# skovaka/UNCALLED

Hardware: AMD Instinct MI355X
Metric: reads_mapped_per_sec (higher is better)
Workload: dtype u64+f32/f64; 1 GPU; E. coli 4.6 Mb synthetic ref (ecoli_syn seed 1), synthetic r9.4.1 reads (3600 bases ~ 32k samples, 10% off-target), all reference defaults; batches_in_flight=2, remapped_reads=0, parallelism=reads sharded over 1 GPU(s), index replicated

## Files before the change

__graft_entry__.py:

```python
import os
import shutil
import subprocess
import sys
from pathlib import Path

ROOT = Path(__file__).resolve().parent
PKG = ROOT / "uncalled_amd"
CSRC = PKG / "csrc"
LIB = ROOT / "uncalled_amd" / "libuncalled_hip.so"
HIP_SOURCES = ["k_events.hip", "k_map.hip", "k_taps.hip", "k_sort.hip", "k_dtw.hip", "k_align.hip", "unc_host.cpp", "unc_dtw.cpp",
               "unc_align.cpp"]
HIPCC_FLAGS = ["--offload-arch=gfx950", "-O3", "-std=c++17", "-ffp-contract=off",
               "-fno-gpu-flush-denormals-to-zero", "-fPIC", "-shared", "-x", "hip"]


def _hipcc():
    for cand in (shutil.which("hipcc"), "/opt/rocm/bin/hipcc"):
        if cand and Path(cand).exists():
            return cand
    raise RuntimeError("hipcc not found")


def _stale(target, sources):
    if not target.exists():
        return True
    t = target.stat().st_mtime
# ... 93 lines not shown
```

include/uncalled_hip.h:

```cpp
#ifndef UNCALLED_HIP_H
#define UNCALLED_HIP_H
#include <stddef.h>
#include <stdint.h>

#ifdef __cplusplus
extern "C" {
#endif

typedef enum {
    UNC_OK = 0,
    UNC_ERR_ARG = -1,
    UNC_ERR_IO = -2,
    UNC_ERR_HIP = -3,
    UNC_ERR_NOMEM = -4,
    UNC_ERR_OVERFLOW = -5
} unc_status_t;

#define UNC_SEED_LEN 22
#define UNC_KLEN 5
#define UNC_NKMER 1024
#define UNC_WINDOW1 3
#define UNC_WINDOW2 6

typedef struct {
// ... 236 lines not shown
    unc_dtw_result_t dtw;
    uint32_t n_events, n_kept;
    float tgt_mean, tgt_stdv;
    float scale, shift;
    uint32_t status, pad;
} unc_align_result_t;
int unc_align_batch(int device, const unc_params_t *params, const unc_align_opts_t *opts, uint32_t n_reads, const int16_t *raw,
                    const uint64_t *offsets, const unc_calib_t *calib, int on_device, uint32_t n_queries, const unc_align_query_t *queries,
                    const uint16_t *kmers, const uint64_t *km_off, uint64_t workspace_bytes, unc_align_result_t *results, float *levels,
                    const uint64_t *lev_off, uint32_t *path, const uint64_t *path_off, void *stream);
int unc_align_last_timing(float *ms4);
void unc_align_model_target(float *mean, float *stdv);

int unc_calib_traffic(int device, uint64_t n_records, int reps);
int unc_calib_chase(int device, const void *base, uint64_t bytes, uint32_t waves, uint32_t steps, float *ms_out);

int unc_detect_events(unc_mapper_t *m, uint32_t n_reads, const int16_t *raw, const uint64_t *offsets,
                      const unc_calib_t *calib, float *means, uint64_t means_cap, uint64_t *means_offsets,
                      unc_evt_info_t *info);
int unc_trace_begin(unc_mapper_t *m, const int16_t *raw, uint32_t n, const unc_calib_t *calib);
int unc_trace_step(unc_mapper_t *m, uint32_t n_events , int *done);
int unc_trace_paths(unc_mapper_t *m, unc_path_t *out, uint32_t cap, uint32_t *n_out);
int unc_trace_clusters(unc_mapper_t *m, unc_cluster_t *out, uint32_t cap, uint32_t *n_out, unc_cluster_t *max_map,
                       float *len_sum, uint32_t *n_lens);
int unc_trace_finish(unc_mapper_t *m, unc_hit_t *hit);

#ifdef __cplusplus
}
#endif
#endif
// ... 1 lines not shown
```

uncalled_amd/csrc/unc_host.cpp:

```cpp
#include <hip/hip_runtime.h>

#include <math.h>
#include <stdarg.h>
#include <stdio.h>
#include <stdlib.h>
#include <string.h>

#include <string>
#include <chrono>
#include <algorithm>
#include <array>
#include <map>
#include <mutex>
#include <utility>
#include <vector>

#include "r94_model_table.h"
#include "unc_dev_types.h"
#include "unc_kernels.h"
#include "unc_host_util.h"

using namespace unc;

static thread_local char g_err[1024] = "";
// ... 128 lines not shown
        if (!fgets(line, sizeof line, fp)) line[0] = 0;
        long long off; int len, n_ambs;
        if (fscanf(fp, "%lld%d%d", &off, &len, &n_ambs) != 3) { fclose(fp); return fail(UNC_ERR_IO, "bad record in %s", fn.c_str()); }
        ix->seqs.push_back(SeqAnn{name, (uint64_t)off, (uint64_t)len});
    }
    fclose(fp);
    return UNC_OK;
}

extern "C" void unc_index_free(unc_index_t *ix) {
    if (!ix) return;
    (void)hipSetDevice(ix->device);
    delete ix;
}

struct PlacementSpacer {
    void *p = nullptr;
    size_t bytes = 0;
    explicit PlacementSpacer(size_t need_after) {
        size_t cap = 64ull << 30;
        if (const char *e = getenv("UNC_PLACEMENT_SPACER_GB")) cap = (size_t)strtoull(e, nullptr, 10) << 30;
        if (need_after < (1ull << 30)) return;
        size_t free_b = 0, total_b = 0;
        if (!cap || hipMemGetInfo(&free_b, &total_b) != hipSuccess) { (void)hipGetLastError(); return; }
        const size_t margin = 16ull << 30;
        if (free_b <= need_after + margin) return;
        const size_t want = std::min(cap, free_b - need_after - margin);
        if (want < (2ull << 30)) return;
        if (hipMalloc(&p, want) != hipSuccess) { p = nullptr; (void)hipGetLastError(); return; }
        bytes = want;
    }
    void release() { if (p) { (void)hipFree(p); p = nullptr; bytes = 0; } }
    ~PlacementSpacer() { release(); }
    PlacementSpacer(const PlacementSpacer &) = delete;
    PlacementSpacer &operator=(const PlacementSpacer &) = delete;
};

extern "C" int unc_index_load(const char *bwa_prefix, const char *idx_preset, int device, unc_index_t **out) {
    if (!bwa_prefix || !out) return fail(UNC_ERR_ARG, "null argument");
    *out = nullptr;
    std::string prefix(bwa_prefix);
    unc_index *ix = new unc_index();
    ix->device = device;
    struct Guard { unc_index *p; ~Guard() { if (p) unc_index_free(p); } } guard{ix};

    std::vector<char> bwt;
    if (!read_file(prefix + ".bwt", bwt) || bwt.size() < 40) return fail(UNC_ERR_IO, "failed to load BWA index: %s.bwt", bwa_prefix);
    memcpy(&ix->primary, bwt.data(), 8);
    memcpy(&ix->L2[1], bwt.data() + 8, 32);
    ix->seq_len = ix->L2[4];
    const size_t n_words = (bwt.size() - 40) / 4;
    const uint64_t n = ix->seq_len;
// ... 6 lines not shown
    memcpy(&sa_primary, sa.data(), 8);
    memcpy(&sa_intv, sa.data() + 40, 8);
    memcpy(&sa_seq_len, sa.data() + 48, 8);
    if (sa_primary != ix->primary || sa_seq_len != n || sa_intv != 32) return fail(UNC_ERR_IO, "%s.sa does not match the .bwt (interval must be 32)", bwa_prefix);
    const uint64_t n_sa = (n + 32) / 32;
    if (sa.size() != 56 + (n_sa - 1) * 8) return fail(UNC_ERR_IO, "%s.sa: unexpected size", bwa_prefix);

    int rc = parse_ann(prefix + ".ann", ix);
    if (rc) return rc;
    rc = parse_uncl(prefix + ".uncl", idx_preset ? idx_preset : "default", ix->thresholds);
    if (rc) return rc;
    build_model(ix);

    HIPCHK(hipSetDevice(device));
    const size_t bwt_bytes = ((n_words * 4 + 63) / 64 + 1) * 64;
    PlacementSpacer spacer(bwt_bytes + n_sa * 8 + ((size_t)n_words * 16 + 2) / 2 * 12 + (size_t)n_words * 2 + (64u << 20));
    HIPCHK(ix->d_bwt.alloc(bwt_bytes / 4));
    HIPCHK(hipMemset(ix->d_bwt.p, 0, bwt_bytes));
    HIPCHK(hipMemcpy(ix->d_bwt.p, bwt.data() + 40, n_words * 4, hipMemcpyHostToDevice));
    HIPCHK(ix->d_sa.alloc(n_sa));
    {
        std::vector<uint64_t> h(n_sa);
        h[0] = ~0ull;
        memcpy(h.data() + 1, sa.data() + 56, (n_sa - 1) * 8);
        HIPCHK(hipMemcpy(ix->d_sa.p, h.data(), n_sa * 8, hipMemcpyHostToDevice));
    }
    HIPCHK(ix->d_kmer_ranges.alloc(2 * NKMER));
    HIPCHK(ix->d_model.alloc(3 * NKMER));
    HIPCHK(hipMemcpy(ix->d_model.p, ix->model.data(), 3 * NKMER * 4, hipMemcpyHostToDevice));
    {
        std::vector<float> m4(4 * NKMER, 0.0f);
        for (int k = 0; k < NKMER; ++k) { m4[4 * k] = ix->model[k]; m4[4 * k + 1] = ix->model[NKMER + k]; m4[4 * k + 2] = ix->model[2 * NKMER + k]; }
        HIPCHK(ix->d_model4.alloc(4 * NKMER));
        HIPCHK(hipMemcpy(ix->d_model4.p, m4.data(), 4 * NKMER * 4, hipMemcpyHostToDevice));
    }
    ix->device_bytes = bwt_bytes + n_sa * 8 + 2 * NKMER * 8 + 3 * NKMER * 4;

    DevIndex &d = ix->dev;
    d.bwt = ix->d_bwt.p; d.sa = ix->d_sa.p; d.kmer_ranges = ix->d_kmer_ranges.p; d.model = ix->d_model.p; d.model4 = ix->d_model4.p;
    d.primary = ix->primary; d.seq_len = n;
    for (int i = 0; i < 5; ++i) d.L2[i] = ix->L2[i];
    memcpy(d.thresholds, ix->thresholds, sizeof d.thresholds);

    d.sa_dense = nullptr;
    {
        const char *env = getenv("UNC_DENSE_SA");
        size_t free_b = 0, total_b = 0;
        (void)hipMemGetInfo(&free_b, &total_b);
        free_b += spacer.bytes;
        const size_t need = ((n + 2) / 2) * 12 + 16;
        if (!(env && env[0] == '0') && need < free_b / 2) {
            HIPCHK(ix->d_sa_dense.alloc(need));
            uint64_t *const dense = reinterpret_cast<uint64_t *>(ix->d_sa_dense.p);
            launch_dense_sa(d, dense, nullptr);
            HIPCHK(hipGetLastError());
            HIPCHK(hipDeviceSynchronize());
            {
                DevBuf<uint32_t> d_bad;
                uint32_t bad = 0;
                HIPCHK(d_bad.alloc(1));
                HIPCHK(hipMemset(d_bad.p, 0, 4));
                launch_dense_sa_check(d, dense, 16384, d_bad.p, nullptr);
                HIPCHK(hipGetLastError());
                HIPCHK(hipMemcpy(&bad, d_bad.p, 4, hipMemcpyDeviceToHost));
                if (bad) return fail(UNC_ERR_HIP, "dense SA self-check failed on %u of 16384 probe rows", bad);
            }
            d.sa_dense = dense;
            ix->device_bytes += need;
        }
    }
    d.fm32 = nullptr;
    const char *fm32_env = getenv("UNC_FM32");
    if (n < 0xFFFFFF00ull && !(fm32_env && fm32_env[0] == '0')) {
        const uint32_t n_blk = (uint32_t)((n + 63) / 64 + 1);
        HIPCHK(ix->d_fm32.alloc((size_t)n_blk * 8));
        launch_build_fm32(d, ix->d_fm32.p, n_blk, nullptr);
        HIPCHK(hipGetLastError());
        HIPCHK(hipDeviceSynchronize());
        d.fm32 = ix->d_fm32.p;
        DevBuf<uint32_t> d_bad;
        uint32_t bad = 0;
        HIPCHK(d_bad.alloc(1));
        HIPCHK(hipMemset(d_bad.p, 0, 4));
        launch_fm32_check(d, 16384, d_bad.p, nullptr);
        HIPCHK(hipGetLastError());
        HIPCHK(hipMemcpy(&bad, d_bad.p, 4, hipMemcpyDeviceToHost));
        if (bad) return fail(UNC_ERR_HIP, "32-bit rank table self-check failed on %u of 16384 probe steps", bad);
        ix->device_bytes += (size_t)n_blk * 32;
    }
    launch_kmer_ranges(d, ix->d_kmer_ranges.p, nullptr);
// ... 118 lines not shown
    HIPCHK(l.alloc(n)); HIPCHK(o.alloc((size_t)n * NKMER));
    HIPCHK(hipMemcpy(l.p, levels, n * 4, hipMemcpyHostToDevice));
    launch_match_probs(ix->dev, n, l.p, o.p, nullptr);
    HIPCHK(hipGetLastError());
    HIPCHK(hipDeviceSynchronize());
    HIPCHK(hipMemcpy(out, o.p, (size_t)n * NKMER * 4, hipMemcpyDeviceToHost));
    return UNC_OK;
}

struct Scratch { DevBuf<char> mem; DevScratch v{}; };
struct Pool { DevBuf<char> nodes; DevBuf<PoolQueue> q; DevBuf<SchedCell> cells; DevPool v{}; };
struct Sched { DevBuf<SchedCtl> ctl; DevBuf<SchedCell> free_cells, park_cells; DevSched v{}; };

struct unc_mapper {
    const unc_index *ix = nullptr;
    unc_params_t P;
    uint32_t n_slots = 0, n_waves = 0, slice_events = 1024, ev_rpw = 64;
    Sched sched;
    Scratch sc;
    uint64_t device_bytes = 0;
    hipStream_t stream = nullptr;
    hipEvent_t ev[3] = {nullptr, nullptr, nullptr};
    double win_start_ms = 0, win_end_ms = 0;
    float ms_events = 0, ms_map = 0;
    double wave_busy = 0;
    float wall_khz = 0;
    bool profile = false;
    Pool pool;
    bool pool_auto = false;
    uint32_t pool_floor = 16, pool_created = 0, pool_hw_last = 0, pool_hw_max = 0, pool_resizes = 0;
// ... 58 lines not shown
    if (off >= (1ull << 32)) return fail(UNC_ERR_ARG, "per-read scratch of %llu bytes does not fit 32-bit offsets (max_clusters %u)", (unsigned long long)off, max_clusters);
    sc.off_paths = (uint32_t)o_paths; sc.off_levels = (uint32_t)o_levels; sc.off_order = (uint32_t)o_order; sc.off_keys = (uint32_t)o_keys;
    sc.off_seedp = (uint32_t)o_seedp; sc.off_tasks = (uint32_t)o_tasks; sc.off_cl_dir = (uint32_t)o_cld; sc.off_cl_chunks = (uint32_t)o_clc;
    sc.off_state = (uint32_t)o_state;
    sc.off_streams = (uint32_t)o_streams; sc.off_info = (uint32_t)o_info; sc.off_tmp = (uint32_t)o_tmp;
    sc.slot_bytes = off;
    return UNC_OK;
}

static uint64_t scratch_slot_bytes(const unc_params_t &P, uint32_t max_clusters, uint32_t max_seed_paths, const DevIndex &dix) {
    DevScratch t;
    return scratch_layout(t, P, max_clusters, max_seed_paths, dix) == UNC_OK ? t.slot_bytes : ~0ull;
}

static int alloc_scratch(Scratch &s, const unc_params_t &P, size_t n_slots, uint32_t max_clusters, uint32_t max_seed_paths,
                         size_t *bytes_out, const DevIndex &dix) {
    DevScratch &sc = s.v;
    int rc = scratch_layout(sc, P, max_clusters, max_seed_paths, dix);
    if (rc) return rc;
    const size_t bytes = (size_t)n_slots * sc.slot_bytes;
    HIPCHK(s.mem.alloc(bytes));
    sc.base = s.mem.p;
    HIPCHK(hipMemset2D(sc.base + sc.off_state, sc.slot_bytes, 0, sizeof(SlotState), n_slots));
    if (bytes_out) *bytes_out = bytes;
    return UNC_OK;
}

static uint32_t xcd_count(int device) {
    static std::mutex mu;
    static std::map<int, uint32_t> known;
    std::lock_guard<std::mutex> lk(mu);
    auto it = known.find(device);
    if (it != known.end()) return it->second;
    uint32_t n = 1;
    DevBuf<uint32_t> d;
    constexpr uint32_t NB = 256;
// ... 5 lines not shown
            for (uint32_t i = 0; i < NB; ++i) seen |= 1u << (h[i] & 15u);
            n = (uint32_t)__builtin_popcount(seen);
            if (seen != (n >= 32 ? ~0u : (1u << n) - 1u)) n = 1;
        }
    }
    (void)hipGetLastError();
    known[device] = n;
    return n;
}

static int alloc_pool(Pool &p, uint32_t n_chunks, size_t *bytes_out) {
    p = Pool{};
    uint32_t cap = 64;
    while (cap < n_chunks) cap <<= 1;
    p.v.cap_mask = cap - 1; p.v.n_chunks = n_chunks;
    HIPCHK(p.nodes.alloc((size_t)n_chunks * POOL_CHUNK_BYTES));
    HIPCHK(p.q.alloc(1));
    HIPCHK(p.cells.alloc(cap));
    p.v.nodes = p.nodes.p; p.v.q = p.q.p; p.v.cells = p.cells.p;
    launch_pool_init(p.v, nullptr);
    HIPCHK(hipGetLastError());
    HIPCHK(hipDeviceSynchronize());
    if (bytes_out) *bytes_out += (size_t)n_chunks * POOL_CHUNK_BYTES + (size_t)cap * sizeof(SchedCell);
    return UNC_OK;
}

static SlotState *slot_state(const DevScratch &sc, size_t slot) { return reinterpret_cast<SlotState *>(sc.base + slot * sc.slot_bytes + sc.off_state); }

extern "C" void unc_mapper_free(unc_mapper_t *m) {
    if (!m) return;
    (void)hipSetDevice(m->ix->device);
    for (auto &e : m->ev) if (e) (void)hipEventDestroy(e);
    if (m->stream) (void)hipStreamDestroy(m->stream);
    delete m;
}

static hipEvent_t g_ref_event = nullptr;
static std::mutex g_ref_mutex;
static int ref_event(hipEvent_t *out) {
    std::lock_guard<std::mutex> lock(g_ref_mutex);
    if (!g_ref_event) {
        HIPCHK(hipEventCreate(&g_ref_event));
        HIPCHK(hipEventRecord(g_ref_event, nullptr));
        HIPCHK(hipEventSynchronize(g_ref_event));
    }
    *out = g_ref_event;
    return UNC_OK;
}
extern "C" int unc_mapper_create(const unc_index_t *ix, const unc_params_t *p, const unc_mapper_opts_t *opts, unc_mapper_t **out) {
    if (!ix || !p || !out) return fail(UNC_ERR_ARG, "null argument");
    *out = nullptr;
    if (p->seed_len != UNC_SEED_LEN) return fail(UNC_ERR_ARG, "seed_len must be %d", UNC_SEED_LEN);
    if (p->window_length1 != UNC_WINDOW1 || p->window_length2 != UNC_WINDOW2) return fail(UNC_ERR_ARG, "event windows must be %d/%d", UNC_WINDOW1, UNC_WINDOW2);
    if (p->max_paths == 0 || p->max_paths > 65535) return fail(UNC_ERR_ARG, "max_paths must be in 1..65535");
    if (p->max_rep_copy > (uint32_t)MAX_REP_COPY_LIMIT) return fail(UNC_ERR_ARG, "max_rep_copy must be <= %d", MAX_REP_COPY_LIMIT);
    if (p->max_consec_stay > 255) return fail(UNC_ERR_ARG, "max_consec_stay must be <= 255");
    if (p->max_events > 65535) return fail(UNC_ERR_ARG, "max_events must be <= 65535");
    HIPCHK(hipSetDevice(ix->device));
    unc_mapper *m = new unc_mapper();
    struct Guard { unc_mapper *p; ~Guard() { if (p) unc_mapper_free(p); } } guard{m};
    m->ix = ix;
    m->P = *p;
    uint32_t n_slots = opts ? opts->n_slots : 0, n_waves = opts ? opts->n_waves : 0;
    if (n_waves == 0) {
        hipDeviceProp_t prop;
        HIPCHK(hipGetDeviceProperties(&prop, ix->device));
        n_waves = (uint32_t)prop.multiProcessorCount * map_kernel_waves_per_cu();
        if (n_slots && n_slots < n_waves) n_waves = n_slots;
    }
    if (n_slots == 0) {
        size_t free_b = 0, total_b = 0;
        HIPCHK(hipMemGetInfo(&free_b, &total_b));
        const uint32_t msp0 = (opts && opts->max_seed_paths) ? opts->max_seed_paths : 2 * p->max_paths;
        const uint32_t mcl0 = (opts && opts->max_clusters) ? opts->max_clusters : (1u << 20);
        const size_t per_slot = scratch_slot_bytes(*p, mcl0, msp0, ix->dev);
        size_t want = (size_t)n_waves * 3, fit = free_b / 3 / per_slot;
        n_slots = (uint32_t)(want < fit ? want : fit);
        if (n_slots > 512) n_slots -= n_slots % 512;
        if (n_slots < n_waves) n_slots = n_waves;
    }
    if (n_slots < n_waves) n_waves = n_slots;
    m->n_slots = n_slots;
    m->n_waves = n_waves;
    m->slice_events = (opts && opts->slice_events) ? opts->slice_events : 1024;
    m->ev_rpw = (opts && opts->events_reads_per_wave) ? opts->events_reads_per_wave : 64;
    if (m->ev_rpw > (uint32_t)WAVE) return fail(UNC_ERR_ARG, "events_reads_per_wave must be in 1..64");
    size_t bytes = 0;
    const uint32_t msp = (opts && opts->max_seed_paths) ? opts->max_seed_paths : 2 * p->max_paths;
    const uint32_t mcl = (opts && opts->max_clusters) ? opts->max_clusters : (1u << 20);
    const size_t pool_per_slot = ix->seq_len >= (1ull << 31) ? 32 : ix->seq_len >= (1ull << 26) ? 24 : 8;
    const size_t pool_want = ((opts && opts->pool_chunks) ? (size_t)opts->pool_chunks : (size_t)n_slots * pool_per_slot) * POOL_CHUNK_BYTES;
    PlacementSpacer spacer((size_t)n_slots * scratch_slot_bytes(*p, mcl, msp, ix->dev) + pool_want);
    int rc_ = alloc_scratch(m->sc, *p, n_slots, mcl, msp, &bytes, ix->dev);
    if (rc_) return rc_;
    HIPCHK(m->d_next.alloc(16));
    {
        uint32_t n_chunks = opts ? opts->pool_chunks : 0;
        if (n_chunks == 0) {
            size_t free_b = 0, total_b = 0;
            HIPCHK(hipMemGetInfo(&free_b, &total_b));
            free_b += spacer.bytes;
            const size_t chunk_bytes = POOL_CHUNK_BYTES;
            const size_t per_slot = pool_per_slot;
            const size_t want = (size_t)n_slots * per_slot;
            n_chunks = (uint32_t)std::max<size_t>(16, std::min<size_t>(want, free_b / 5 * 3 / chunk_bytes));
            m->pool_auto = true;
            m->pool_floor = std::max<uint32_t>(16, std::min<uint32_t>(n_slots, n_chunks));
            m->pool_created = n_chunks;
        }
        int rc2 = alloc_pool(m->pool, n_chunks, &bytes);
        if (rc2) return rc2;
    }
    spacer.release();
    if (n_slots > n_waves) {
        uint32_t parts = (opts && opts->sched_parts) ? opts->sched_parts : xcd_count(ix->device);
        if (parts > SCHED_MAX_PARTS || parts == 0 || n_slots % parts || n_slots / parts < 64 || (opts && opts->sched_parts > 1 && opts->sched_parts != xcd_count(ix->device))) {
            if (opts && opts->sched_parts > 1) return fail(UNC_ERR_ARG, "sched_parts: 0, 1 or the device's number of XCDs (%u), dividing n_slots into shares of 64 or more", xcd_count(ix->device));
            parts = 1;
        }
        const uint32_t spp = n_slots / parts;
        uint32_t cap = 64;
        while (cap < spp) cap <<= 1;
        m->sched.v.cap_mask = cap - 1; m->sched.v.n_slots = n_slots; m->sched.v.n_parts = parts;
        HIPCHK(m->sched.ctl.alloc(1));
        HIPCHK(m->sched.free_cells.alloc((size_t)parts * cap));
        HIPCHK(m->sched.park_cells.alloc((size_t)parts * cap));
        m->sched.v.ctl = m->sched.ctl.p; m->sched.v.free_cells = m->sched.free_cells.p; m->sched.v.park_cells = m->sched.park_cells.p;
        bytes += sizeof(SchedCtl) + 2 * (size_t)parts * cap * sizeof(SchedCell);
// ... 120 lines not shown
    return UNC_OK;
}

static int pool_fit(unc_mapper *m, bool went_dry, uint32_t n_reads) {
    if (!m->pool_auto) return UNC_OK;
    const uint64_t cur = m->pool.v.n_chunks;
    uint64_t target = cur;
    if (went_dry) {
        target = std::max<uint64_t>(std::max<uint64_t>(cur * 2, m->pool_created), 4ull * m->pool_hw_max);
    } else if (n_reads >= m->n_slots) {
        const uint64_t need = std::max<uint64_t>(m->pool_floor, 4ull * m->pool_hw_max);
        if (need * 2 < cur) target = need;
    }
    if (target > cur) {
        size_t free_b = 0, total_b = 0;
        HIPCHK(hipMemGetInfo(&free_b, &total_b));
        const uint64_t most = (free_b + cur * (uint64_t)POOL_CHUNK_BYTES) / 5 * 3 / POOL_CHUNK_BYTES;
        target = std::max(cur, std::min(target, most));
    }
    if (target == cur) return UNC_OK;
    HIPCHK(hipDeviceSynchronize());
    Pool fresh;
    size_t bytes = 0;
    if (target < cur) {
        if (alloc_pool(fresh, (uint32_t)target, &bytes) != UNC_OK) { (void)hipGetLastError(); return UNC_OK; }
    } else {
        m->pool = Pool{};
        if (alloc_pool(fresh, (uint32_t)target, &bytes) != UNC_OK) {
            (void)hipGetLastError();
            target = cur;
            int rc = alloc_pool(fresh, (uint32_t)cur, &bytes);
// ... 106 lines not shown
static void classify(const unc_mapper *m, uint32_t i, std::vector<uint32_t> &dry, std::vector<uint32_t> &full) {
    const uint32_t stt = m->h_results[i].status;
    if (stt & UNC_READ_POOL_DRY) dry.push_back(i);
    else if (stt & UNC_READ_CLUSTER_OVERFLOW) full.push_back(i);
}

static int ensure_big_scratch(unc_mapper *m, uint64_t cap, size_t want) {
    if (m->big.v.max_clusters == cap && (m->big_slots >= want || m->big_at_limit)) return UNC_OK;
    m->big = Scratch{};
    m->big_slots = 0;
    size_t free_b = 0, total_b = 0;
    HIPCHK(hipMemGetInfo(&free_b, &total_b));
    const size_t per_slot = scratch_slot_bytes(m->P, (uint32_t)cap, m->sc.v.max_seed_paths, m->ix->dev);
    const size_t fit = std::max<size_t>(1, free_b / 4 / per_slot);
    const size_t n = std::min(want, fit);
    int rc = alloc_scratch(m->big, m->P, n, (uint32_t)cap, m->sc.v.max_seed_paths, nullptr, m->ix->dev);
    if (rc) { m->big = Scratch{}; return rc; }
    m->big_slots = n; m->big_at_limit = n == fit;
    return UNC_OK;
}

static int resolve_overflows(unc_mapper *m, const std::vector<uint32_t> *subset, bool *pool_went_dry) {
    std::vector<uint32_t> dry, full, work;
    if (subset) { for (uint32_t i : *subset) classify(m, i, dry, full); }
    else { for (uint32_t i = 0; i < m->pend.n_reads; ++i) classify(m, i, dry, full); }
    m->remap_reads += (uint32_t)(dry.size() + full.size());
    if (!dry.empty()) *pool_went_dry = true;
    const auto t_redo = std::chrono::steady_clock::now();
    uint64_t cap = m->sc.v.max_clusters;
    size_t limit = m->n_waves;
    while (!dry.empty() || !full.empty()) {
// ... 515 lines not shown
    unc_evt_info_t inf;
    HIPCHK(hipMemcpy(&inf, m->d_info.p, sizeof inf, hipMemcpyDeviceToHost));
    DevResult res;
    memset(&res, 0, sizeof res);
    res.done = s.done; res.status = s.status; res.event_i = s.event_i; res.cluster = s.max_map;
    res.n_nbr = s.n_nbr; res.n_sa = s.n_sa; res.n_lf = s.n_lf;
    fill_hit(m->ix, m->P, res, inf, m->trace_n, hit);
    m->trace_active = false;
    return UNC_OK;
}

struct RtHostChan { int state = 0;  uint32_t number = 0, chunk_count = 0; uint64_t raw_len = 0; };

struct unc_rt {
    const unc_index *ix = nullptr;
    unc_params_t P;
    uint32_t n_channels = 0;
    uint32_t team = 8;
    Scratch sc;
    Pool pool;
    DevBuf<RtChan> d_chans;
    DevBuf<float> d_ring;
    DevBuf<RtChunkDesc> d_desc;
    DevBuf<unc_evt_info_t> d_info;
    DevBuf<uint32_t> d_ring0, d_newread, d_slotmap, d_next;
    DevBuf<uint64_t> d_moff;
    DevBuf<DevResult> d_results;
    DevBuf<int16_t> d_raw;
    uint64_t device_bytes = 0;
    hipStream_t stream = nullptr;
// ... 5 lines not shown
    std::vector<unc_evt_info_t> h_info;
    bool profile = false;
    uint64_t cyc_sum[12] = {0};
};

extern "C" void unc_rt_free(unc_rt_t *rt) {
    if (!rt) return;
    if (rt->profile) {
        static const char *names[12] = {"probs", "extend_rest", "sort", "walk", "sources", "sa", "add_seed", "rest", "e1_parents", "e2_fm", "e3_slots", "e4_children"};
        double tot = 0;
        for (uint64_t c : rt->cyc_sum) tot += (double)c;
        fprintf(stderr, "UNC_RT_PROFILE phase cycle shares of the finished reads:");
        for (int i = 0; i < 12; ++i) fprintf(stderr, " %s %.3f", names[i], tot > 0 ? (double)rt->cyc_sum[i] / tot : 0.0);
        fprintf(stderr, "\n");
    }
    (void)hipSetDevice(rt->ix->device);
    for (auto &e : rt->ev) if (e) (void)hipEventDestroy(e);
    if (rt->stream) (void)hipStreamDestroy(rt->stream);
    delete rt;
}

template <class T> static int alloc_zeroed(DevBuf<T> &buf, size_t count, size_t *bytes) {
    HIPCHK(buf.alloc(count));
    HIPCHK(hipMemset(buf.p, 0, count * sizeof(T)));
    *bytes += count * sizeof(T);
    return UNC_OK;
}

extern "C" int unc_rt_create(const unc_index_t *ix, const unc_params_t *p, uint32_t n_channels, unc_rt_t **out) {
    if (!ix || !p || !out || n_channels == 0) return fail(UNC_ERR_ARG, "bad argument");
    *out = nullptr;
    if (p->seed_len != UNC_SEED_LEN || p->window_length1 != UNC_WINDOW1 || p->window_length2 != UNC_WINDOW2)
        return fail(UNC_ERR_ARG, "seed_len/window lengths must be %d/%d/%d", UNC_SEED_LEN, UNC_WINDOW1, UNC_WINDOW2);
    if (p->max_paths == 0 || p->max_paths > 65535 || p->max_rep_copy > (uint32_t)MAX_REP_COPY_LIMIT || p->max_consec_stay > 255 ||
        p->max_events > 65535)
        return fail(UNC_ERR_ARG, "unsupported parameter value");
    if (!(p->chunk_time > 0.0f) || !(p->sample_rate > 0.0f) || (double)p->chunk_time * (double)p->sample_rate > 2.0 * (double)NORM_LEN)
        return fail(UNC_ERR_ARG, "chunk_time * sample_rate = %.0f samples: chunks of more than %u samples are not supported (mapper.cpp:336-351, "
                                 "the #SKIP branch of the reference, is out of scope)", (double)p->chunk_time * (double)p->sample_rate, 2u * NORM_LEN);
    HIPCHK(hipSetDevice(ix->device));
    unc_rt *rt = new unc_rt();
    struct Guard { unc_rt *p; ~Guard() { if (p) unc_rt_free(p); } } guard{rt};
    rt->ix = ix; rt->P = *p; rt->n_channels = n_channels;
    { const char *e = getenv("UNC_RT_PROFILE"); rt->profile = e && e[0] == '1'; }
    {
        const char *e = getenv("UNC_RT_TEAM");
#ifdef LANESIM
        if (!e) e = getenv("UNC_SIM_RT_TEAM");
#endif
        const long v = e ? atol(e) : 8;
        rt->team = v >= 8 ? 8u : v >= 4 ? 4u : v >= 2 ? 2u : 1u;
    }
    const size_t S = n_channels;
    size_t bytes = 0;
    {
        PlacementSpacer spacer(S * scratch_slot_bytes(*p, 1u << 20, 2 * p->max_paths, ix->dev) + S * 64 * (size_t)POOL_CHUNK_BYTES);
        int rc = alloc_scratch(rt->sc, *p, S, 1u << 20, 2 * p->max_paths, &bytes, ix->dev);
        if (rc) return rc;
        HIPCHK(hipMemset(rt->sc.v.base, 0, bytes));
        size_t per_ch = ix->seq_len >= (1ull << 26) ? 64 : 16;
        size_t n_chunks = S * per_ch;
        {
            size_t free_b = 0, total_b = 0;
            HIPCHK(hipMemGetInfo(&free_b, &total_b));
            free_b += spacer.bytes;
            const size_t fit = free_b / 5 * 3 / POOL_CHUNK_BYTES;
            if (n_chunks > fit) {
                const size_t floor_chunks = std::max<size_t>(64, (size_t)S * 4);
                const size_t clamped = std::max(fit, floor_chunks);
                fprintf(stderr, "Warning: realtime node pool clamped from %zu to %zu chunks (%.1f GB of HBM free)\n", n_chunks, clamped, (double)free_b / 1e9);
                n_chunks = clamped;
            }
        }
        n_chunks = std::max<size_t>(64, n_chunks);
        if (const char *e = getenv("UNC_RT_POOL_CHUNKS")) { const long v = atol(e); if (v > 0) n_chunks = (size_t)v; }
        rc = alloc_pool(rt->pool, (uint32_t)n_chunks, &bytes);
        if (rc) return rc;
    }
    {
        int rc = UNC_OK;
// ... 232 lines not shown
    DevBuf<uint8_t> d_pac;
    DevBuf<uint64_t> d_pos, d_rem, d_out;
    DevBuf<uint32_t> d_len;
    HIPCHK(d_pac.alloc(pac.size() + 16)); HIPCHK(d_pos.alloc(n)); HIPCHK(d_rem.alloc(n)); HIPCHK(d_out.alloc((size_t)n * cap)); HIPCHK(d_len.alloc(n));
    HIPCHK(hipMemcpy(d_pac.p, pac.data(), pac.size(), hipMemcpyHostToDevice));
    HIPCHK(hipMemcpy(d_pos.p, pos.data(), (size_t)n * 8, hipMemcpyHostToDevice));
    HIPCHK(hipMemcpy(d_rem.p, remain.data(), (size_t)n * 8, hipMemcpyHostToDevice));
    HIPCHK(hipMemset(d_out.p, 0, (size_t)n * cap * 8));
    launch_self_align(ix->dev, d_pac.p, n, d_pos.p, d_rem.p, d_out.p, cap, d_len.p, nullptr);
    HIPCHK(hipGetLastError());
    HIPCHK(hipDeviceSynchronize());
    HIPCHK(hipMemcpy(lens, d_out.p, (size_t)n * cap * 8, hipMemcpyDeviceToHost));
    HIPCHK(hipMemcpy(full_len, d_len.p, (size_t)n * 4, hipMemcpyDeviceToHost));
    return UNC_OK;
}
```

uncalled_amd/csrc/unc_host_util.h:

```cpp
#pragma once
#include <hip/hip_runtime.h>
#include <stddef.h>

#include "../../include/uncalled_hip.h"

namespace unc {
int fail(int code, const char *fmt, ...);
}

#define HIPCHK(expr)                                                                                         \
    do {                                                                                                     \
        hipError_t e_ = (expr);                                                                              \
        if (e_ != hipSuccess) return unc::fail(UNC_ERR_HIP, "%s failed: %s (%s:%d)", #expr, hipGetErrorString(e_), \
                                               __FILE__, __LINE__);                                          \
    } while (0)

template <class T> struct DevBuf {
    T *p = nullptr;
    size_t cap = 0;
    DevBuf() = default;
    DevBuf(const DevBuf &) = delete;
    DevBuf &operator=(const DevBuf &) = delete;
    DevBuf(DevBuf &&o) noexcept : p(o.p), cap(o.cap) { o.p = nullptr; o.cap = 0; }
    DevBuf &operator=(DevBuf &&o) noexcept {
        if (this != &o) { release(); p = o.p; cap = o.cap; o.p = nullptr; o.cap = 0; }
        return *this;
    }
    ~DevBuf() { release(); }
    void release() { if (p) (void)hipFree(p); p = nullptr; cap = 0; }
    hipError_t alloc(size_t n, size_t slack = 0) {
        release();
        if (!n) n = 1;
        const hipError_t e = hipMalloc((void **)&p, (n + slack) * sizeof(T));
        if (e != hipSuccess) { p = nullptr; return e; }
        cap = n;
        return hipSuccess;
    }
    hipError_t reserve(size_t n, size_t slack = 0) { return n <= cap ? hipSuccess : alloc(n, slack); }
};
```

Measured before the change: 23850 reads/s.

## Replace placement spacer with a VMM-backed device arena for index and scratch buffers

Adds a per-device arena allocator that reserves a large virtual address range and maps physical chunks via hipMemCreate/hipMemMap, with a hipMalloc block fallback. Index tables, mapper scratch, and node pools now come from this arena, and the old PlacementSpacer hack, which pushed allocations to particular HBM addresses, is removed. The aim is contiguous 2 MB-aligned placement of hot buffers to cut TLB and fragmentation cost. The trade-off is allocator complexity and a device synchronize on every arena free.

```diff
diff --git a/__graft_entry__.py b/__graft_entry__.py
--- a/__graft_entry__.py
+++ b/__graft_entry__.py
@@ -9,7 +9,7 @@
 CSRC = PKG / "csrc"
 LIB = ROOT / "uncalled_amd" / "libuncalled_hip.so"
 HIP_SOURCES = ["k_events.hip", "k_map.hip", "k_taps.hip", "k_sort.hip", "k_dtw.hip", "k_align.hip", "unc_host.cpp", "unc_dtw.cpp",
-               "unc_align.cpp"]
+               "unc_align.cpp", "unc_arena.cpp"]
 HIPCC_FLAGS = ["--offload-arch=gfx950", "-O3", "-std=c++17", "-ffp-contract=off",
                "-fno-gpu-flush-denormals-to-zero", "-fPIC", "-shared", "-x", "hip"]
 
diff --git a/include/uncalled_hip.h b/include/uncalled_hip.h
--- a/include/uncalled_hip.h
+++ b/include/uncalled_hip.h
@@ -274,6 +274,9 @@
 
 int unc_calib_traffic(int device, uint64_t n_records, int reps);
 int unc_calib_chase(int device, const void *base, uint64_t bytes, uint32_t waves, uint32_t steps, float *ms_out);
+int unc_arena_stats(int device, uint64_t *out6);
+int unc_arena_contains(int device, const void *p, uint64_t bytes);
+int unc_arena_release(int device);
 
 int unc_detect_events(unc_mapper_t *m, uint32_t n_reads, const int16_t *raw, const uint64_t *offsets,
                       const unc_calib_t *calib, float *means, uint64_t means_cap, uint64_t *means_offsets,
diff --git a/uncalled_amd/csrc/unc_arena.cpp b/uncalled_amd/csrc/unc_arena.cpp
--- /dev/null
+++ b/uncalled_amd/csrc/unc_arena.cpp
@@ -0,0 +1,258 @@
+#include "unc_host_util.h"
+
+#include <stdlib.h>
+#include <string.h>
+
+#include <iterator>
+#include <map>
+#include <mutex>
+#include <vector>
+
+#if !defined(LANESIM) && !defined(UNC_ARENA_NO_VMM)
+#define UNC_ARENA_VMM 1
+#endif
+
+namespace {
+
+struct Range {
+    size_t bytes;
+    bool used;
+    uint32_t seg;
+};
+
+struct Piece {
+    char *base;
+    size_t bytes;
+    bool mapped;
+#ifdef UNC_ARENA_VMM
+    hipMemGenericAllocationHandle_t handle;
+#endif
+};
+
+struct Arena {
+    std::map<uintptr_t, Range> ranges;
+    std::vector<Piece> pieces;
+    char *va = nullptr;
+    size_t va_bytes = 0, va_used = 0, gran = 0;
+    bool vmm_tried = false, vmm_ok = false;
+    uint32_t next_seg = 1;
+    size_t held = 0, in_use = 0, n_used = 0;
+};
+
+std::mutex g_mu;
+std::map<int, Arena> &arenas() {
+    static std::map<int, Arena> *a = new std::map<int, Arena>();
+    return *a;
+}
+
+enum class Mode { OFF, MAPPED, BLOCKS };
+Mode mode() {
+    const char *e = getenv("UNC_ARENA");
+#ifdef LANESIM
+    if (!e || !e[0]) return Mode::OFF;
+#else
+    if (!e || !e[0]) return Mode::MAPPED;
+#endif
+    if (e[0] == '0') return Mode::OFF;
+    if (!strcmp(e, "blocks")) return Mode::BLOCKS;
+    return Mode::MAPPED;
+}
+
+size_t round_up(size_t v, size_t a) { return (v + a - 1) / a * a; }
+
+std::map<uintptr_t, Range>::iterator mapped_tail(Arena &A) {
+    if (!A.va || !A.va_used) return A.ranges.end();
+    auto it = A.ranges.upper_bound((uintptr_t)A.va + A.va_used - 1);
+    if (it == A.ranges.begin()) return A.ranges.end();
+    --it;
+    if (it->second.seg != 0 || it->second.used || it->first + it->second.bytes != (uintptr_t)A.va + A.va_used) return A.ranges.end();
+    return it;
+}
+
+#ifdef UNC_ARENA_VMM
+hipError_t grow_mapped(Arena &A, int device, size_t more) {
+    hipMemAllocationProp prop;
+    memset(&prop, 0, sizeof prop);
+    prop.type = hipMemAllocationTypePinned;
+    prop.location.type = hipMemLocationTypeDevice;
+    prop.location.id = device;
+    if (!A.vmm_tried) {
+        A.vmm_tried = true;
+        size_t gran = 0, free_b = 0, total_b = 0;
+        hipError_t e = hipMemGetAllocationGranularity(&gran, &prop, hipMemAllocationGranularityRecommended);
+        if (e != hipSuccess || gran == 0) return e != hipSuccess ? e : hipErrorNotSupported;
+        e = hipMemGetInfo(&free_b, &total_b);
+        if (e != hipSuccess) return e;
+        A.gran = round_up(gran, unc::ARENA_ALIGN);
+        size_t want = round_up(2 * total_b, 1ull << 30);
+        void *va = nullptr;
+        while (want >= (1ull << 30) && (e = hipMemAddressReserve(&va, want, unc::ARENA_ALIGN, nullptr, 0)) != hipSuccess) { va = nullptr; want /= 2; }
+        if (!va) return e != hipSuccess ? e : hipErrorOutOfMemory;
+        if ((uintptr_t)va % unc::ARENA_ALIGN) { (void)hipMemAddressFree(va, want); return hipErrorNotSupported; }
+        A.va = (char *)va; A.va_bytes = want; A.va_used = 0; A.vmm_ok = true;
+    }
+    if (!A.vmm_ok) return hipErrorNotSupported;
+    more = round_up(more, A.gran);
+    if (more > A.va_bytes - A.va_used) return hipErrorOutOfMemory;
+    Piece pc;
+    pc.base = A.va + A.va_used; pc.bytes = more; pc.mapped = true;
+    hipError_t e = hipMemCreate(&pc.handle, more, &prop, 0);
+    if (e != hipSuccess) return e;
+    e = hipMemMap(pc.base, more, 0, pc.handle, 0);
+    if (e != hipSuccess) { (void)hipMemRelease(pc.handle); return e; }
+    hipMemAccessDesc acc;
+    memset(&acc, 0, sizeof acc);
+    acc.location = prop.location;
+    acc.flags = hipMemAccessFlagsProtReadWrite;
+    e = hipMemSetAccess(pc.base, more, &acc, 1);
+    if (e != hipSuccess) { (void)hipMemUnmap(pc.base, more); (void)hipMemRelease(pc.handle); return e; }
+    auto tail = mapped_tail(A);
+    if (tail != A.ranges.end()) tail->second.bytes += more;
+    else A.ranges[(uintptr_t)pc.base] = Range{more, false, 0};
+    A.va_used += more;
+    A.held += more;
+    A.pieces.push_back(pc);
+    return hipSuccess;
+}
+#endif
+
+hipError_t grow_block(Arena &A, size_t need, std::map<uintptr_t, Range>::iterator *out) {
+    void *raw = nullptr;
+    const hipError_t e = hipMalloc(&raw, need + unc::ARENA_ALIGN);
+    if (e != hipSuccess) return e;
+    Piece pc;
+    memset(&pc, 0, sizeof pc);
+    pc.base = (char *)raw; pc.bytes = need + unc::ARENA_ALIGN; pc.mapped = false;
+    A.pieces.push_back(pc);
+    A.held += need;
+    *out = A.ranges.emplace(round_up((uintptr_t)raw, unc::ARENA_ALIGN), Range{need, false, A.next_seg++}).first;
+    return hipSuccess;
+}
+
+void *take(Arena &A, std::map<uintptr_t, Range>::iterator it, size_t need) {
+    Range &r = it->second;
+    if (r.bytes > need) A.ranges[it->first + need] = Range{r.bytes - need, false, r.seg};
+    r.bytes = need; r.used = true;
+    A.in_use += need; A.n_used++;
+    return (void *)it->first;
+}
+
+}
+
+bool unc::arena_enabled() { return mode() != Mode::OFF; }
+
+hipError_t unc::arena_alloc(void **p, size_t bytes) {
+    *p = nullptr;
+    int device = 0;
+    hipError_t e = hipGetDevice(&device);
+    if (e != hipSuccess) return e;
+    const size_t need = round_up(bytes ? bytes : 1, ARENA_ALIGN);
+    std::lock_guard<std::mutex> lk(g_mu);
+    Arena &A = arenas()[device];
+    for (auto it = A.ranges.begin(); it != A.ranges.end(); ++it)
+        if (!it->second.used && it->second.bytes >= need) { *p = take(A, it, need); return hipSuccess; }
+#ifdef UNC_ARENA_VMM
+    if (mode() == Mode::MAPPED) {
+        auto tail = mapped_tail(A);
+        const size_t have = tail != A.ranges.end() ? tail->second.bytes : 0;
+        if (grow_mapped(A, device, need - have) == hipSuccess) {
+            tail = mapped_tail(A);
+            if (tail != A.ranges.end() && tail->second.bytes >= need) { *p = take(A, tail, need); return hipSuccess; }
+        }
+        (void)hipGetLastError();
+    }
+#endif
+    std::map<uintptr_t, Range>::iterator it;
+    e = grow_block(A, need, &it);
+    if (e != hipSuccess) return e;
+    *p = take(A, it, need);
+    return hipSuccess;
+}
+
+bool unc::arena_free(void *p) {
+    if (!p) return false;
+    std::lock_guard<std::mutex> lk(g_mu);
+    for (auto &da : arenas()) {
+        Arena &A = da.second;
+        auto it = A.ranges.find((uintptr_t)p);
+        if (it == A.ranges.end() || !it->second.used) continue;
+        it->second.used = false;
+        A.in_use -= it->second.bytes; A.n_used--;
+        auto next = std::next(it);
+        if (next != A.ranges.end() && !next->second.used && next->second.seg == it->second.seg && it->first + it->second.bytes == next->first) {
+            it->second.bytes += next->second.bytes;
+            A.ranges.erase(next);
+        }
+        if (it != A.ranges.begin()) {
+            auto prev = std::prev(it);
+            if (!prev->second.used && prev->second.seg == it->second.seg && prev->first + prev->second.bytes == it->first) {
+                prev->second.bytes += it->second.bytes;
+                A.ranges.erase(it);
+            }
+        }
+        return true;
+    }
+    return false;
+}
+
+size_t unc::arena_free_bytes() {
+    int device = 0;
+    if (hipGetDevice(&device) != hipSuccess) { (void)hipGetLastError(); return 0; }
+    std::lock_guard<std::mutex> lk(g_mu);
+    auto it = arenas().find(device);
+    return it == arenas().end() ? 0 : it->second.held - it->second.in_use;
+}
+
+hipError_t unc::arena_mem_get_info(size_t *free_b, size_t *total_b) {
+    const hipError_t e = hipMemGetInfo(free_b, total_b);
+    if (e == hipSuccess) *free_b += arena_free_bytes();
+    return e;
+}
+
+extern "C" int unc_arena_stats(int device, uint64_t *out6) {
+    if (!out6) return unc::fail(UNC_ERR_ARG, "null argument");
+    memset(out6, 0, 6 * sizeof *out6);
+    std::lock_guard<std::mutex> lk(g_mu);
+    auto it = arenas().find(device);
+    if (it == arenas().end()) return UNC_OK;
+    const Arena &A = it->second;
+    out6[0] = A.held; out6[1] = A.in_use; out6[2] = A.n_used; out6[3] = A.pieces.size();
+    out6[4] = (!A.pieces.empty() && A.pieces[0].mapped) ? 1 : 0;
+    out6[5] = A.ranges.size() - A.n_used;
+    return UNC_OK;
+}
+
+extern "C" int unc_arena_contains(int device, const void *p, uint64_t bytes) {
+    std::lock_guard<std::mutex> lk(g_mu);
+    auto da = arenas().find(device);
+    if (da == arenas().end() || !p) return 0;
+    const Arena &A = da->second;
+    auto it = A.ranges.upper_bound((uintptr_t)p);
+    if (it == A.ranges.begin()) return 0;
+    --it;
+    return it->second.used && bytes <= it->second.bytes && (uintptr_t)p - it->first <= it->second.bytes - bytes;
+}
+
+extern "C" int unc_arena_release(int device) {
+    std::lock_guard<std::mutex> lk(g_mu);
+    auto da = arenas().find(device);
+    if (da == arenas().end()) return UNC_OK;
+    Arena &A = da->second;
+    if (A.n_used) return unc::fail(UNC_ERR_ARG, "unc_arena_release: %zu ranges of device %d's arena are in use", A.n_used, device);
+    int prev = 0;
+    const bool have_prev = hipGetDevice(&prev) == hipSuccess;
+    HIPCHK(hipSetDevice(device));
+    for (Piece &pc : A.pieces) {
+#ifdef UNC_ARENA_VMM
+        if (pc.mapped) { (void)hipMemUnmap(pc.base, pc.bytes); (void)hipMemRelease(pc.handle); continue; }
+#endif
+        (void)hipFree(pc.base);
+    }
+#ifdef UNC_ARENA_VMM
+    if (A.va) (void)hipMemAddressFree(A.va, A.va_bytes);
+#endif
+    (void)hipGetLastError();
+    arenas().erase(da);
+    if (have_prev) (void)hipSetDevice(prev);
+    return UNC_OK;
+}
diff --git a/uncalled_amd/csrc/unc_arena.h b/uncalled_amd/csrc/unc_arena.h
--- /dev/null
+++ b/uncalled_amd/csrc/unc_arena.h
@@ -0,0 +1,16 @@
+#pragma once
+#include <hip/hip_runtime.h>
+#include <stddef.h>
+#include <stdint.h>
+
+#include "../../include/uncalled_hip.h"
+
+namespace unc {
+constexpr size_t ARENA_ALIGN = 2ull << 20;
+
+bool arena_enabled();
+hipError_t arena_alloc(void **p, size_t bytes);
+bool arena_free(void *p);
+size_t arena_free_bytes();
+hipError_t arena_mem_get_info(size_t *free_b, size_t *total_b);
+}
diff --git a/uncalled_amd/csrc/unc_host.cpp b/uncalled_amd/csrc/unc_host.cpp
--- a/uncalled_amd/csrc/unc_host.cpp
+++ b/uncalled_amd/csrc/unc_host.cpp
@@ -166,28 +166,6 @@
     delete ix;
 }
 
-struct PlacementSpacer {
-    void *p = nullptr;
-    size_t bytes = 0;
-    explicit PlacementSpacer(size_t need_after) {
-        size_t cap = 64ull << 30;
-        if (const char *e = getenv("UNC_PLACEMENT_SPACER_GB")) cap = (size_t)strtoull(e, nullptr, 10) << 30;
-        if (need_after < (1ull << 30)) return;
-        size_t free_b = 0, total_b = 0;
-        if (!cap || hipMemGetInfo(&free_b, &total_b) != hipSuccess) { (void)hipGetLastError(); return; }
-        const size_t margin = 16ull << 30;
-        if (free_b <= need_after + margin) return;
-        const size_t want = std::min(cap, free_b - need_after - margin);
-        if (want < (2ull << 30)) return;
-        if (hipMalloc(&p, want) != hipSuccess) { p = nullptr; (void)hipGetLastError(); return; }
-        bytes = want;
-    }
-    void release() { if (p) { (void)hipFree(p); p = nullptr; bytes = 0; } }
-    ~PlacementSpacer() { release(); }
-    PlacementSpacer(const PlacementSpacer &) = delete;
-    PlacementSpacer &operator=(const PlacementSpacer &) = delete;
-};
-
 extern "C" int unc_index_load(const char *bwa_prefix, const char *idx_preset, int device, unc_index_t **out) {
     if (!bwa_prefix || !out) return fail(UNC_ERR_ARG, "null argument");
     *out = nullptr;
@@ -224,11 +202,10 @@
 
     HIPCHK(hipSetDevice(device));
     const size_t bwt_bytes = ((n_words * 4 + 63) / 64 + 1) * 64;
-    PlacementSpacer spacer(bwt_bytes + n_sa * 8 + ((size_t)n_words * 16 + 2) / 2 * 12 + (size_t)n_words * 2 + (64u << 20));
-    HIPCHK(ix->d_bwt.alloc(bwt_bytes / 4));
+    HIPCHK(ix->d_bwt.alloc_arena(bwt_bytes / 4));
     HIPCHK(hipMemset(ix->d_bwt.p, 0, bwt_bytes));
     HIPCHK(hipMemcpy(ix->d_bwt.p, bwt.data() + 40, n_words * 4, hipMemcpyHostToDevice));
-    HIPCHK(ix->d_sa.alloc(n_sa));
+    HIPCHK(ix->d_sa.alloc_arena(n_sa));
     {
         std::vector<uint64_t> h(n_sa);
         h[0] = ~0ull;
@@ -256,11 +233,10 @@
     {
         const char *env = getenv("UNC_DENSE_SA");
         size_t free_b = 0, total_b = 0;
-        (void)hipMemGetInfo(&free_b, &total_b);
-        free_b += spacer.bytes;
+        (void)arena_mem_get_info(&free_b, &total_b);
         const size_t need = ((n + 2) / 2) * 12 + 16;
         if (!(env && env[0] == '0') && need < free_b / 2) {
-            HIPCHK(ix->d_sa_dense.alloc(need));
+            HIPCHK(ix->d_sa_dense.alloc_arena(need));
             uint64_t *const dense = reinterpret_cast<uint64_t *>(ix->d_sa_dense.p);
             launch_dense_sa(d, dense, nullptr);
             HIPCHK(hipGetLastError());
@@ -283,7 +259,7 @@
     const char *fm32_env = getenv("UNC_FM32");
     if (n < 0xFFFFFF00ull && !(fm32_env && fm32_env[0] == '0')) {
         const uint32_t n_blk = (uint32_t)((n + 63) / 64 + 1);
-        HIPCHK(ix->d_fm32.alloc((size_t)n_blk * 8));
+        HIPCHK(ix->d_fm32.alloc_arena((size_t)n_blk * 8));
         launch_build_fm32(d, ix->d_fm32.p, n_blk, nullptr);
         HIPCHK(hipGetLastError());
         HIPCHK(hipDeviceSynchronize());
@@ -432,6 +408,7 @@
 
 struct unc_mapper {
     const unc_index *ix = nullptr;
+    int device = 0;
     unc_params_t P;
     uint32_t n_slots = 0, n_waves = 0, slice_events = 1024, ev_rpw = 64;
     Sched sched;
@@ -520,12 +497,12 @@
 }
 
 static int alloc_scratch(Scratch &s, const unc_params_t &P, size_t n_slots, uint32_t max_clusters, uint32_t max_seed_paths,
-                         size_t *bytes_out, const DevIndex &dix) {
+                         size_t *bytes_out, const DevIndex &dix, bool arena) {
     DevScratch &sc = s.v;
     int rc = scratch_layout(sc, P, max_clusters, max_seed_paths, dix);
     if (rc) return rc;
     const size_t bytes = (size_t)n_slots * sc.slot_bytes;
-    HIPCHK(s.mem.alloc(bytes));
+    HIPCHK(arena ? s.mem.alloc_arena(bytes) : s.mem.alloc(bytes));
     sc.base = s.mem.p;
     HIPCHK(hipMemset2D(sc.base + sc.off_state, sc.slot_bytes, 0, sizeof(SlotState), n_slots));
     if (bytes_out) *bytes_out = bytes;
@@ -561,7 +538,7 @@
     uint32_t cap = 64;
     while (cap < n_chunks) cap <<= 1;
     p.v.cap_mask = cap - 1; p.v.n_chunks = n_chunks;
-    HIPCHK(p.nodes.alloc((size_t)n_chunks * POOL_CHUNK_BYTES));
+    HIPCHK(p.nodes.alloc_arena((size_t)n_chunks * POOL_CHUNK_BYTES));
     HIPCHK(p.q.alloc(1));
     HIPCHK(p.cells.alloc(cap));
     p.v.nodes = p.nodes.p; p.v.q = p.q.p; p.v.cells = p.cells.p;
@@ -576,7 +553,7 @@
 
 extern "C" void unc_mapper_free(unc_mapper_t *m) {
     if (!m) return;
-    (void)hipSetDevice(m->ix->device);
+    (void)hipSetDevice(m->device);
     for (auto &e : m->ev) if (e) (void)hipEventDestroy(e);
     if (m->stream) (void)hipStreamDestroy(m->stream);
     delete m;
@@ -607,6 +584,7 @@
     unc_mapper *m = new unc_mapper();
     struct Guard { unc_mapper *p; ~Guard() { if (p) unc_mapper_free(p); } } guard{m};
     m->ix = ix;
+    m->device = ix->device;
     m->P = *p;
     uint32_t n_slots = opts ? opts->n_slots : 0, n_waves = opts ? opts->n_waves : 0;
     if (n_waves == 0) {
@@ -617,7 +595,7 @@
     }
     if (n_slots == 0) {
         size_t free_b = 0, total_b = 0;
-        HIPCHK(hipMemGetInfo(&free_b, &total_b));
+        HIPCHK(arena_mem_get_info(&free_b, &total_b));
         const uint32_t msp0 = (opts && opts->max_seed_paths) ? opts->max_seed_paths : 2 * p->max_paths;
         const uint32_t mcl0 = (opts && opts->max_clusters) ? opts->max_clusters : (1u << 20);
         const size_t per_slot = scratch_slot_bytes(*p, mcl0, msp0, ix->dev);
@@ -636,29 +614,26 @@
     const uint32_t msp = (opts && opts->max_seed_paths) ? opts->max_seed_paths : 2 * p->max_paths;
     const uint32_t mcl = (opts && opts->max_clusters) ? opts->max_clusters : (1u << 20);
     const size_t pool_per_slot = ix->seq_len >= (1ull << 31) ? 32 : ix->seq_len >= (1ull << 26) ? 24 : 8;
-    const size_t pool_want = ((opts && opts->pool_chunks) ? (size_t)opts->pool_chunks : (size_t)n_slots * pool_per_slot) * POOL_CHUNK_BYTES;
-    PlacementSpacer spacer((size_t)n_slots * scratch_slot_bytes(*p, mcl, msp, ix->dev) + pool_want);
-    int rc_ = alloc_scratch(m->sc, *p, n_slots, mcl, msp, &bytes, ix->dev);
+    int rc_ = alloc_scratch(m->sc, *p, n_slots, mcl, msp, &bytes, ix->dev, true);
     if (rc_) return rc_;
     HIPCHK(m->d_next.alloc(16));
     {
         uint32_t n_chunks = opts ? opts->pool_chunks : 0;
         if (n_chunks == 0) {
             size_t free_b = 0, total_b = 0;
-            HIPCHK(hipMemGetInfo(&free_b, &total_b));
-            free_b += spacer.bytes;
+            HIPCHK(arena_mem_get_info(&free_b, &total_b));
             const size_t chunk_bytes = POOL_CHUNK_BYTES;
             const size_t per_slot = pool_per_slot;
             const size_t want = (size_t)n_slots * per_slot;
             n_chunks = (uint32_t)std::max<size_t>(16, std::min<size_t>(want, free_b / 5 * 3 / chunk_bytes));
             m->pool_auto = true;
             m->pool_floor = std::max<uint32_t>(16, std::min<uint32_t>(n_slots, n_chunks));
+            if (const char *e = getenv("UNC_POOL_CHUNKS")) { const long v = atol(e); if (v > 0) { n_chunks = (uint32_t)v; m->pool_floor = std::min(m->pool_floor, n_chunks); } }
             m->pool_created = n_chunks;
         }
         int rc2 = alloc_pool(m->pool, n_chunks, &bytes);
         if (rc2) return rc2;
     }
-    spacer.release();
     if (n_slots > n_waves) {
         uint32_t parts = (opts && opts->sched_parts) ? opts->sched_parts : xcd_count(ix->device);
         if (parts > SCHED_MAX_PARTS || parts == 0 || n_slots % parts || n_slots / parts < 64 || (opts && opts->sched_parts > 1 && opts->sched_parts != xcd_count(ix->device))) {
@@ -809,7 +784,7 @@
     }
     if (target > cur) {
         size_t free_b = 0, total_b = 0;
-        HIPCHK(hipMemGetInfo(&free_b, &total_b));
+        HIPCHK(arena_mem_get_info(&free_b, &total_b));
         const uint64_t most = (free_b + cur * (uint64_t)POOL_CHUNK_BYTES) / 5 * 3 / POOL_CHUNK_BYTES;
         target = std::max(cur, std::min(target, most));
     }
@@ -946,7 +921,7 @@
     const size_t per_slot = scratch_slot_bytes(m->P, (uint32_t)cap, m->sc.v.max_seed_paths, m->ix->dev);
     const size_t fit = std::max<size_t>(1, free_b / 4 / per_slot);
     const size_t n = std::min(want, fit);
-    int rc = alloc_scratch(m->big, m->P, n, (uint32_t)cap, m->sc.v.max_seed_paths, nullptr, m->ix->dev);
+    int rc = alloc_scratch(m->big, m->P, n, (uint32_t)cap, m->sc.v.max_seed_paths, nullptr, m->ix->dev, false);
     if (rc) { m->big = Scratch{}; return rc; }
     m->big_slots = n; m->big_at_limit = n == fit;
     return UNC_OK;
@@ -1492,6 +1467,7 @@
 
 struct unc_rt {
     const unc_index *ix = nullptr;
+    int device = 0;
     unc_params_t P;
     uint32_t n_channels = 0;
     uint32_t team = 8;
@@ -1527,7 +1503,7 @@
         for (int i = 0; i < 12; ++i) fprintf(stderr, " %s %.3f", names[i], tot > 0 ? (double)rt->cyc_sum[i] / tot : 0.0);
         fprintf(stderr, "\n");
     }
-    (void)hipSetDevice(rt->ix->device);
+    (void)hipSetDevice(rt->device);
     for (auto &e : rt->ev) if (e) (void)hipEventDestroy(e);
     if (rt->stream) (void)hipStreamDestroy(rt->stream);
     delete rt;
@@ -1554,7 +1530,7 @@
     HIPCHK(hipSetDevice(ix->device));
     unc_rt *rt = new unc_rt();
     struct Guard { unc_rt *p; ~Guard() { if (p) unc_rt_free(p); } } guard{rt};
-    rt->ix = ix; rt->P = *p; rt->n_channels = n_channels;
+    rt->ix = ix; rt->device = ix->device; rt->P = *p; rt->n_channels = n_channels;
     { const char *e = getenv("UNC_RT_PROFILE"); rt->profile = e && e[0] == '1'; }
     {
         const char *e = getenv("UNC_RT_TEAM");
@@ -1567,16 +1543,14 @@
     const size_t S = n_channels;
     size_t bytes = 0;
     {
-        PlacementSpacer spacer(S * scratch_slot_bytes(*p, 1u << 20, 2 * p->max_paths, ix->dev) + S * 64 * (size_t)POOL_CHUNK_BYTES);
-        int rc = alloc_scratch(rt->sc, *p, S, 1u << 20, 2 * p->max_paths, &bytes, ix->dev);
+        int rc = alloc_scratch(rt->sc, *p, S, 1u << 20, 2 * p->max_paths, &bytes, ix->dev, true);
         if (rc) return rc;
         HIPCHK(hipMemset(rt->sc.v.base, 0, bytes));
         size_t per_ch = ix->seq_len >= (1ull << 26) ? 64 : 16;
         size_t n_chunks = S * per_ch;
         {
             size_t free_b = 0, total_b = 0;
-            HIPCHK(hipMemGetInfo(&free_b, &total_b));
-            free_b += spacer.bytes;
+            HIPCHK(arena_mem_get_info(&free_b, &total_b));
             const size_t fit = free_b / 5 * 3 / POOL_CHUNK_BYTES;
             if (n_chunks > fit) {
                 const size_t floor_chunks = std::max<size_t>(64, (size_t)S * 4);
@@ -1839,3 +1813,7 @@
     HIPCHK(hipMemcpy(full_len, d_len.p, (size_t)n * 4, hipMemcpyDeviceToHost));
     return UNC_OK;
 }
+
+#ifdef LANESIM
+#include "unc_arena.cpp"
+#endif
diff --git a/uncalled_amd/csrc/unc_host_util.h b/uncalled_amd/csrc/unc_host_util.h
--- a/uncalled_amd/csrc/unc_host_util.h
+++ b/uncalled_amd/csrc/unc_host_util.h
@@ -3,6 +3,7 @@
 #include <stddef.h>
 
 #include "../../include/uncalled_hip.h"
+#include "unc_arena.h"
 
 namespace unc {
 int fail(int code, const char *fmt, ...);
@@ -18,16 +19,20 @@
 template <class T> struct DevBuf {
     T *p = nullptr;
     size_t cap = 0;
+    bool in_arena = false;
     DevBuf() = default;
     DevBuf(const DevBuf &) = delete;
     DevBuf &operator=(const DevBuf &) = delete;
-    DevBuf(DevBuf &&o) noexcept : p(o.p), cap(o.cap) { o.p = nullptr; o.cap = 0; }
+    DevBuf(DevBuf &&o) noexcept : p(o.p), cap(o.cap), in_arena(o.in_arena) { o.p = nullptr; o.cap = 0; o.in_arena = false; }
     DevBuf &operator=(DevBuf &&o) noexcept {
-        if (this != &o) { release(); p = o.p; cap = o.cap; o.p = nullptr; o.cap = 0; }
+        if (this != &o) { release(); p = o.p; cap = o.cap; in_arena = o.in_arena; o.p = nullptr; o.cap = 0; o.in_arena = false; }
         return *this;
     }
     ~DevBuf() { release(); }
-    void release() { if (p) (void)hipFree(p); p = nullptr; cap = 0; }
+    void release() {
+        if (p) { if (in_arena) { (void)hipDeviceSynchronize(); (void)unc::arena_free(p); } else (void)hipFree(p); }
+        p = nullptr; cap = 0; in_arena = false;
+    }
     hipError_t alloc(size_t n, size_t slack = 0) {
         release();
         if (!n) n = 1;
@@ -36,5 +41,14 @@
         cap = n;
         return hipSuccess;
     }
+    hipError_t alloc_arena(size_t n, size_t slack = 0) {
+        if (!unc::arena_enabled()) return alloc(n, slack);
+        release();
+        if (!n) n = 1;
+        const hipError_t e = unc::arena_alloc((void **)&p, (n + slack) * sizeof(T));
+        if (e != hipSuccess) { p = nullptr; return e; }
+        cap = n; in_arena = true;
+        return hipSuccess;
+    }
     hipError_t reserve(size_t n, size_t slack = 0) { return n <= cap ? hipSuccess : alloc(n, slack); }
 };
```

Result: no change. 24340 reads/s (median of 2 runs) (+2.1%).
